# Beryl2000/SE-UNet-AirSeg

Hardware: AMD Instinct MI355X
Metric: voxels/sec SE-UNet fwd+bwd, 128^3 patch (higher is better)
Workload: dtype bf16

## Files before the change

se-unet-airseg_amd/csrc/cat.hip:

```cpp
#include "epilogue.h"
#include <type_traits>

namespace seunet {

template <bool XR>
__device__ __forceinline__ void second_branch(const float (&in8)[8], const float (&wa)[8], const float (&wb)[8], float (&x2)[8]) {
#pragma unroll
  for (int j = 0; j < 8; ++j) x2[j] = XR ? wa[j] * in8[0] + wb[j] * in8[1] : in8[j];
}

template <typename T, int LPV, bool TWO, bool XR>
__global__ void __launch_bounds__(EPI_THREADS)
cat_fwd_kernel(const T* __restrict__ raw, const float* __restrict__ mean, const float* __restrict__ rstd,
               const T* __restrict__ raw2, const float* __restrict__ mean2, const float* __restrict__ rstd2, int C, float slope,
               T* __restrict__ out, long long V, const float* __restrict__ w2x, int xic) {
  SEUNET_EPI_THREAD(LPV);
  float mu[8], rs[8], mu2[8], rs2[8], wa[8], wb[8];
#pragma unroll
  for (int j = 0; j < 8; ++j) {
    mu[j] = mean[n * C + c0 + j]; rs[j] = rstd[n * C + c0 + j];
    mu2[j] = TWO ? mean2[n * C + c0 + j] : 0.f;
    rs2[j] = TWO ? rstd2[n * C + c0 + j] : 0.f;
    wa[j] = XR ? w2x[(c0 + j) * xic] : 0.f;
    wb[j] = (XR && xic > 1) ? w2x[(c0 + j) * xic + 1] : 0.f;
  }
  const long long stride = (long long)P * VPB;
  long long v = (long long)blockIdx.x * VPB + vb;
  Pack8<T> nx, nx2;
  zero8p(nx); zero8p(nx2);
  if (v < V) {
    const long long o = ((long long)n * V + v) * C + c0;
    load8p(raw + o, nx);
    if (TWO) load8p(XR ? raw2 + ((long long)n * V + v) * 8 : raw2 + o, nx2);
  }
  for (; v < V; v += stride) {
    const long long o = ((long long)n * V + v) * C + c0;
    float x[8], in2[8], x2[8], y[8];
    unpack8(nx, x);
    if (TWO) { unpack8(nx2, in2); second_branch<XR>(in2, wa, wb, x2); }
    if (v + stride < V) {
      load8p(raw + o + stride * C, nx);
      if (TWO) load8p(XR ? raw2 + ((long long)n * V + v + stride) * 8 : raw2 + o + stride * C, nx2);
    }
#pragma unroll
    for (int j = 0; j < 8; ++j) y[j] = norm_lrelu(x[j], mu[j], rs[j], slope);
    if (TWO) {
#pragma unroll
      for (int j = 0; j < 8; ++j) y[j] += norm_lrelu(x2[j], mu2[j], rs2[j], slope);
    }
    store8(out + o, y);
  }
}

template <typename T, int LPV>
__global__ void __launch_bounds__(EPI_THREADS)
cat_fwd_pool_kernel(const T* __restrict__ raw, const float* __restrict__ mean, const float* __restrict__ rstd,
                    const T* __restrict__ xin, const float* __restrict__ mean2, const float* __restrict__ rstd2, int C, float slope,
                    T* __restrict__ out, T* __restrict__ pooled, int D, int H, int W, const float* __restrict__ w2x, int xic,
                    unsigned* __restrict__ argmax) {
  SEUNET_EPI_THREAD(LPV);
  float mu[8], rs[8], mu2[8], rs2[8], wa[8], wb[8];
#pragma unroll
  for (int j = 0; j < 8; ++j) {
    mu[j] = mean[n * C + c0 + j]; rs[j] = rstd[n * C + c0 + j];
    mu2[j] = mean2[n * C + c0 + j]; rs2[j] = rstd2[n * C + c0 + j];
    wa[j] = w2x[(c0 + j) * xic];
    wb[j] = xic > 1 ? w2x[(c0 + j) * xic + 1] : 0.f;
  }
  const int Do = D / 2, Ho = H / 2, Wo = W / 2;
  const long long V = (long long)D * H * W, Vo = (long long)Do * Ho * Wo;
  const long long stride = (long long)P * VPB;
  for (long long cv = (long long)blockIdx.x * VPB + vb; cv < Vo; cv += stride) {
    const int xo = (int)(cv % Wo);
    const int yo = (int)((cv / Wo) % Ho);
    const int zo = (int)(cv / ((long long)Wo * Ho));
    const long long v0 = ((long long)(2 * zo) * H + 2 * yo) * W + 2 * xo;
    Pack8<T> px[8], pi[8];
#pragma unroll
    for (int k = 0; k < 8; ++k) {
      const long long v = v0 + ((long long)(k >> 2) * H + ((k >> 1) & 1)) * W + (k & 1);
      load8p(raw + ((long long)n * V + v) * C + c0, px[k]);
      load8p(xin + ((long long)n * V + v) * 8, pi[k]);
    }
    float m[8];
// ... 51 lines not shown
               const T* __restrict__ raw2, const float* __restrict__ mean2, const float* __restrict__ rstd2, int C, float slope,
               const float* __restrict__ m1p, const float* __restrict__ m2p, const float* __restrict__ m1bp,
               const float* __restrict__ m2bp, T* dxhat_out, T* dxhat2_out, double* __restrict__ stat_partial,
               double* __restrict__ stat_partial2, long long V, double* __restrict__ xw_partial, const float* __restrict__ w2x,
               int xic, PoolRef pool, float* __restrict__ gx_out, int gx_acc) {
  static_assert(!XG || (APPLY && XR), "XG: pass B of an XR block only");
  static_assert(!XW || XR, "XW: the weight-gradient sums are formed from the recomputed branch's own input voxel");
  SEUNET_EPI_THREAD(LPV);
  const bool pooled = pool.argmax != nullptr;
  const unsigned* pam = pool.argmax + (long long)n * pool.Vo * (C / 8) + cg;
  const T* pgp = reinterpret_cast<const T*>(pool.g_pool) + (long long)n * pool.Vo * C + c0;
  float mu[8], rs[8], mu2[8], rs2[8], a1[8], a2[8], b1[8], b2[8];
  typedef typename std::conditional<sizeof(T) == 2, float, double>::type SumT;
  SumT s[4][8];
  SumT xw[8][2];
  float wa[8], wb[8];
#pragma unroll
  for (int j = 0; j < 8; ++j) {
    xw[j][0] = xw[j][1] = 0.0;
    wa[j] = XR ? w2x[(c0 + j) * xic] : 0.f;
    wb[j] = (XR && xic > 1) ? w2x[(c0 + j) * xic + 1] : 0.f;
  }
#pragma unroll
  for (int j = 0; j < 8; ++j) {
    mu[j] = mean[n * C + c0 + j]; rs[j] = rstd[n * C + c0 + j];
    mu2[j] = TWO ? mean2[n * C + c0 + j] : 0.f;
    rs2[j] = TWO ? rstd2[n * C + c0 + j] : 0.f;
    a1[j] = APPLY ? m1p[n * C + c0 + j] : 0.f;
    a2[j] = APPLY ? m2p[n * C + c0 + j] : 0.f;
    b1[j] = (APPLY && TWO) ? m1bp[n * C + c0 + j] : 0.f;
    b2[j] = (APPLY && TWO) ? m2bp[n * C + c0 + j] : 0.f;
    s[0][j] = s[1][j] = s[2][j] = s[3][j] = 0.0;
  }
  const long long stride = (long long)P * VPB;
  long long v = (long long)blockIdx.x * VPB + vb;
  Pack8<T> ng, nx, nx2, npg;
  unsigned nam = 0, nkpos = 0;
  zero8p(ng); zero8p(nx); zero8p(nx2); zero8p(npg);
  auto fetch_pool = [&](long long vv) __attribute__((always_inline)) {
    unsigned cv;
    pool_locate(pool, (unsigned)vv, nkpos, cv);
    nam = pam[(long long)cv * (C / 8)];
    load8p(pgp + (long long)cv * C, npg);
  };
  if (v < V) {
    const long long o = ((long long)n * V + v) * C + c0;
    load8p(g_out + o, ng);
    load8p(raw + o, nx);
    if (TWO) load8p(XR ? raw2 + ((long long)n * V + v) * 8 : raw2 + o, nx2);
    if (pooled) fetch_pool(v);
  }
  for (; v < V; v += stride) {
    const long long o = ((long long)n * V + v) * C + c0;
    float gy[8], x[8], in2[8], x2[8], d[8];
    unpack8(ng, gy);
    unpack8(nx, x);
    if (TWO) { unpack8(nx2, in2); second_branch<XR>(in2, wa, wb, x2); }
    if (pooled) {
      float gp[8];
      unpack8(npg, gp);
#pragma unroll
      for (int j = 0; j < 8; ++j) gy[j] += ((nam >> (3 * j)) & 7u) == nkpos ? gp[j] : 0.f;
    }
    if (v + stride < V) {
      load8p(g_out + o + stride * C, ng);
      load8p(raw + o + stride * C, nx);
      if (TWO) load8p(XR ? raw2 + ((long long)n * V + v + stride) * 8 : raw2 + o + stride * C, nx2);
      if (pooled) fetch_pool(v + stride);
    }
#pragma unroll
    for (int j = 0; j < 8; ++j) {
      const float xh = (x[j] - mu[j]) * rs[j];
      d[j] = gy[j] * lrelu_slope(xh, slope);
      if (APPLY) d[j] = rs[j] * (d[j] - a1[j] - xh * a2[j]);
      else { s[0][j] += (SumT)d[j]; s[1][j] += (SumT)d[j] * (SumT)xh; }
    }
    if (TWO) {
      float d2[8];
#pragma unroll
      for (int j = 0; j < 8; ++j) {
        const float xh = (x2[j] - mu2[j]) * rs2[j];
        d2[j] = gy[j] * lrelu_slope(xh, slope);
        if (APPLY) d2[j] = rs2[j] * (d2[j] - b1[j] - xh * b2[j]);
        else { s[2][j] += (SumT)d2[j]; s[3][j] += (SumT)d2[j] * (SumT)xh; }
      }
      if (APPLY && !XR) store8(dxhat2_out + o, d2);
      if (XG) {
        float pa = 0.f, pb = 0.f;
#pragma unroll
        for (int j = 0; j < 8; ++j) { pa = fmaf(d2[j], wa[j], pa); pb = fmaf(d2[j], wb[j], pb); }
#pragma unroll
        for (int off = 1; off < LPV; off <<= 1) { pa += shfl_xor_settled(pa, off); pb += shfl_xor_settled(pb, off); }
        if (cg == 0) {
          float* gp = gx_out + ((long long)n * V + v) * xic;
          gp[0] = gx_acc ? gp[0] + pa : pa;
          if (xic > 1) gp[1] = gx_acc ? gp[1] + pb : pb;
        }
      }
      if (XW && !APPLY) {
#pragma unroll
        for (int j = 0; j < 8; ++j) { xw[j][0] += (SumT)d2[j] * (SumT)in2[0]; xw[j][1] += (SumT)d2[j] * (SumT)in2[1]; }
      }
    }
    if (APPLY) store8(dxhat_out + o, d);
  }
  if (APPLY) return;
  const int wave = threadIdx.x >> 6, lane = threadIdx.x & 63;
  if (XW) {
    __shared__ double redx[4][16][16];
#pragma unroll
    for (int j = 0; j < 8; ++j)
#pragma unroll
      for (int i = 0; i < 2; ++i) {
        const double r = stride_sum_d<LPV>((double)xw[j][i]);
        if (lane < LPV) redx[wave][lane][j * 2 + i] = r;
      }
    __syncthreads();
    double* rec = xw_partial + ((long long)n * P + blockIdx.x) * (C * 2);
    for (int e = threadIdx.x; e < LPV * 16; e += EPI_THREADS) {
      const int gq = e / 16, k = e % 16;
      rec[(gq * 8 + (k >> 1)) * 2 + (k & 1)] = ((redx[0][gq][k] + redx[1][gq][k]) + redx[2][gq][k]) + redx[3][gq][k];
    }
  }
  __shared__ double red[4][16][32];
#pragma unroll
  for (int q = 0; q < 4; ++q)
#pragma unroll
    for (int j = 0; j < 8; ++j) {
      const double r = stride_sum_d<LPV>((double)s[q][j]);
      if (lane < LPV) red[wave][lane][q * 8 + j] = r;
    }
  __syncthreads();
  const long long rec = (long long)n * P + blockIdx.x;
  for (int i = threadIdx.x; i < LPV * 32; i += EPI_THREADS) {
    const int gq = i / 32, k = i % 32, q = k >> 3;
    const double tot = ((red[0][gq][k] + red[1][gq][k]) + red[2][gq][k]) + red[3][gq][k];
    const int c = gq * 8 + (k & 7);
    if (q < 2) stat_partial[(rec * C + c) * 2 + q] = tot;
// ... 248 lines not shown
```

se-unet-airseg_amd/csrc/epilogue.h:

```cpp
#pragma once
#include "seunet_common.h"

namespace seunet {

int epi_partials(Dims d);
int launch_channel_stats(int dtype, const void* t, int C, double* partial, Dims d, hipStream_t s);
int launch_stats_finalize(const double* partial, int slots, int C, int N, long long count,
                          float eps, int mode, float* out_a, float* out_b, hipStream_t s);
struct NormIn { const void* raw; const float* mean; const float* rstd; };
struct SseParams {
  const float* w_se;
  const float* w_se2;
  const float* w_side;
  const float* b_side;
  float slope;
};
struct GateBlock { NormIn a; int C; SseParams p; };
struct SseHead {
  float* side_out;
  float* level_map;
  int level_accumulate;
  const float* head_w;
  const float* drop;
  int drop_stride;
// ... 24 lines not shown
  const float* w2;
  int in_channel;
};
struct CatBlock { NormIn a; Branch2 b; int C; float slope; };
struct PoolOut { void* pooled; unsigned* argmax; };
struct PoolGrad { const unsigned* argmax; const void* g_pool; };
struct CatSums {
  double* stat_partial;
  double* stat_partial2;
  double* xw_partial;
};
struct CatApply {
  const float *m1, *m2, *m1b, *m2b;
  void* dx;
  void* dx2;
  float* gx_out;
  int gx_acc;
};
int launch_cat_fwd(int dtype, const CatBlock& b, void* out, const PoolOut& pool, Dims d, hipStream_t s);
int launch_cat_bwd_sums(int dtype, const CatBlock& b, const void* g_out, const PoolGrad& pool, const CatSums& out, Dims d,
                        hipStream_t s);
int launch_cat_bwd_apply(int dtype, const CatBlock& b, const void* g_out, const PoolGrad& pool, const CatApply& io, Dims d,
                         hipStream_t s);
int xbranch_moment_slots(Dims d);
int launch_xbranch_moments(int dtype, const void* x_in, double* partial, Dims d, hipStream_t s);
int launch_xbranch_stats(const double* partial, int slots, const float* w2, int C, int in_channel, int N, long long count,
                         float eps, float* mean2, float* rstd2, double* moments_out, hipStream_t s);
int launch_cat_xgrad_finalize(const double* xw_partial, const double* stat_partial2, int slots, const double* moments, const float* w2,
                              int C, int in_channel, int N, float eps, float* dw, hipStream_t s);
int launch_xbranch_values(int dtype, const void* x_in, const float* w2, int C, int in_channel, float* out_ncdhw, Dims d, hipStream_t s);

#ifdef __HIPCC__
static constexpr int EPI_THREADS = 256;

template <typename T> __device__ __forceinline__ float round_to(float v) {
  if constexpr (sizeof(T) == 4) return v;
  else return unpack_lo<T>(pack2<T>(v, 0.f));
}

template <typename T> __device__ __forceinline__ float gate_sigmoid(float z) {
  if constexpr (sizeof(T) == 4) return 1.f / (1.f + expf(-z));
  else return __builtin_amdgcn_rcpf(1.f + __builtin_amdgcn_exp2f(-1.44269504088896341f * z));
}

#define SEUNET_EPI_THREAD(LPV)                                \
  const int n = blockIdx.y, P = gridDim.x;                    \
  const int cg = threadIdx.x % LPV, vb = threadIdx.x / LPV;   \
  constexpr int VPB = EPI_THREADS / LPV;                      \
  const int c0 = cg * 8

__device__ __forceinline__ float lrelu(float xh, float slope) { return xh > 0.f ? xh : xh * slope; }
__device__ __forceinline__ float norm_lrelu(float x, float mu, float rs, float slope) { return lrelu((x - mu) * rs, slope); }
__device__ __forceinline__ float lrelu_slope(float xh, float slope) { return xh > 0.f ? 1.f : slope; }

template <typename E, int K> __device__ __forceinline__ E wave4_sum(const E (&red)[4][16][K], int g, int k) {
  return ((red[0][g][k] + red[1][g][k]) + red[2][g][k]) + red[3][g][k];
}
template <typename E, int K> __device__ __forceinline__ E wave4_sum(const E (&red)[4][K], int k) {
  return ((red[0][k] + red[1][k]) + red[2][k]) + red[3][k];
}
template <typename E> __device__ __forceinline__ E wave4_sum(const E (&w)[4]) { return ((w[0] + w[1]) + w[2]) + w[3]; }

template <int K> __device__ __forceinline__ void block_sum(const double (&s)[K], double (&red)[4][K]) {
  const int wave = threadIdx.x >> 6, lane = threadIdx.x & 63;
#pragma unroll
  for (int k = 0; k < K; ++k) {
    double r = s[k];
#pragma unroll
    for (int off = 32; off >= 1; off >>= 1) r += shfl_xor_settled(r, off);
    if (lane == 0) red[wave][k] = r;
  }
  __syncthreads();
}

__device__ __forceinline__ void stats_finalize_body(int idx, const double* __restrict__ partial, int slots, int C, double inv_count,
                                                    float eps, int mode, float* __restrict__ out_a, float* __restrict__ out_b) {
  const int n = idx / C, c = idx % C;
  double s1 = 0.0, s2 = 0.0;
  for (int p = threadIdx.x; p < slots; p += 256) {
    const double* q = partial + (((long long)n * slots + p) * C + c) * 2;
    s1 += q[0];
    s2 += q[1];
// ... 43 lines not shown
```

se-unet-airseg_amd/csrc/epilogue.hip:

```cpp
#include "epilogue.h"

namespace seunet {

int epi_partials(Dims d) {
  long long v = d.vox();
  long long p = v / 128;
  if (p < 1) p = 1;
  if (p > 256) p = 256;
  const long long n = d.N > 0 ? d.N : 1, round = 3 * 256;
  if (n * p >= round) {
    const long long q = (n * p / round) * round / n;
    if (q >= 1) p = q;
  }
  return (int)p;
}

template <typename T, int LPV>
__global__ void __launch_bounds__(EPI_THREADS)
channel_stats_kernel(const T* __restrict__ t, int C, double* __restrict__ partial, long long V) {
  SEUNET_EPI_THREAD(LPV);
  double s1[8], s2[8];
#pragma unroll
  for (int j = 0; j < 8; ++j) { s1[j] = 0.0; s2[j] = 0.0; }
  for (long long v = (long long)blockIdx.x * VPB + vb; v < V; v += (long long)P * VPB) {
    float x[8];
    load8(t + ((long long)n * V + v) * C + c0, x);
#pragma unroll
    for (int j = 0; j < 8; ++j) { s1[j] += (double)x[j]; s2[j] += (double)x[j] * (double)x[j]; }
  }
  __shared__ double red[4][16][16];
  const int wave = threadIdx.x >> 6, lane = threadIdx.x & 63;
#pragma unroll
  for (int j = 0; j < 8; ++j) {
    double a = stride_sum_d<LPV>(s1[j]), b = stride_sum_d<LPV>(s2[j]);
    if (lane < LPV) { red[wave][lane][j] = a; red[wave][lane][8 + j] = b; }
  }
  __syncthreads();
  for (int i = threadIdx.x; i < LPV * 16; i += EPI_THREADS) {
    const int g = i / 16, k = i % 16;
    const double tot = wave4_sum(red, g, k);
    const int c = g * 8 + (k & 7);
    partial[(((long long)n * P + blockIdx.x) * C + c) * 2 + (k >> 3)] = tot;
  }
}

__global__ void __launch_bounds__(256)
stats_finalize_kernel(const double* __restrict__ partial, int slots, int C, int N, double inv_count,
                      float eps, int mode, float* __restrict__ out_a, float* __restrict__ out_b) {
  stats_finalize_body(blockIdx.x, partial, slots, C, inv_count, eps, mode, out_a, out_b);
}

int launch_channel_stats(int dtype, const void* t, int C, double* partial, Dims d, hipStream_t s) {
  if (int e = check_c(C)) return e;
  dim3 grid(epi_partials(d), d.N);
  SEUNET_LPV_SWITCH(C / 8, {
    SEUNET_DTYPE_SWITCH(dtype, channel_stats_kernel<T, LPV><<<grid, EPI_THREADS, 0, s>>>((const T*)t, C, partial, d.vox()));
  });
  SEUNET_LAUNCH_CHECK();
  return 0;
}

int launch_stats_finalize(const double* partial, int slots, int C, int N, long long count, float eps,
// ... 8 lines not shown
```

se-unet-airseg_amd/csrc/gate.hip:

```cpp
#include "epilogue.h"

namespace seunet {

template <typename T, int LPV, bool G2>
__global__ void __launch_bounds__(EPI_THREADS)
sse_fwd_kernel(const T* __restrict__ raw, const float* __restrict__ mean, const float* __restrict__ rstd, int C, SseParams p,
               T* __restrict__ e_out, SseHead head, long long V) {
  SEUNET_EPI_THREAD(LPV);
  float mu[8], rs[8], wse[8], wse2[8], w20[8], w21[8];
#pragma unroll
  for (int j = 0; j < 8; ++j) {
    mu[j] = mean[n * C + c0 + j];
    rs[j] = rstd[n * C + c0 + j];
    wse[j] = p.w_se[c0 + j];
    wse2[j] = G2 ? p.w_se2[c0 + j] : 0.f;
    w20[j] = p.w_side[c0 + j];
    w21[j] = p.w_side[C + c0 + j];
  }
  const float b20 = p.b_side[0], b21 = p.b_side[1], slope = p.slope;
  const bool want_side = head.side_out != nullptr || head.level_map != nullptr;
  float hw0 = 0.f, hw1 = 0.f;
  if (head.level_map) {
    hw0 = head.head_w[0] * (head.drop ? head.drop[n * head.drop_stride + 0] : 1.f);
    hw1 = head.head_w[1] * (head.drop ? head.drop[n * head.drop_stride + 1] : 1.f);
  }
  const long long stride = (long long)P * VPB;
  long long v = (long long)blockIdx.x * VPB + vb;
  Pack8<T> nx;
  zero8p(nx);
  if (v < V) load8p(raw + ((long long)n * V + v) * C + c0, nx);
  for (; v < V; v += stride) {
    const long long vi = (long long)n * V + v;
    float x[8], a[8], e[8];
    unpack8(nx, x);
    if (v + stride < V) load8p(raw + (vi + stride) * C + c0, nx);
    float d1 = 0.f;
#pragma unroll
    for (int j = 0; j < 8; ++j) {
      a[j] = norm_lrelu(x[j], mu[j], rs[j], slope);
      d1 += wse[j] * a[j];
    }
    const float g1 = gate_sigmoid<T>(group_sum<LPV>(d1));
    float d2 = 0.f;
#pragma unroll
    for (int j = 0; j < 8; ++j) {
      e[j] = a[j] * g1;
      d2 += wse2[j] * e[j];
    }
    if (G2) {
      const float g2 = gate_sigmoid<T>(group_sum<LPV>(d2));
#pragma unroll
      for (int j = 0; j < 8; ++j) e[j] *= g2;
    }
    store8(e_out + vi * C + c0, e);
    if (want_side) {
      float s0 = 0.f, s1 = 0.f;
#pragma unroll
      for (int j = 0; j < 8; ++j) { s0 += w20[j] * e[j]; s1 += w21[j] * e[j]; }
      s0 = group_sum<LPV>(s0) + b20;
      s1 = group_sum<LPV>(s1) + b21;
      if (cg == 0) {
        if (head.side_out) { head.side_out[vi * 2] = s0; head.side_out[vi * 2 + 1] = s1; }
        if (head.level_map) {
          const float t = hw0 * s0 + hw1 * s1;
          head.level_map[vi] = head.level_accumulate ? head.level_map[vi] + t : t;
        }
      }
    }
  }
}

template <typename T, int LPV, bool G2, bool APPLY, bool LEVEL>
__global__ void __launch_bounds__(EPI_THREADS, (APPLY || G2) ? 1 : 3)
sse_bwd_kernel(const T* __restrict__ raw, const float* __restrict__ mean, const float* __restrict__ rstd, int C, SseParams p,
               SseBwdIn g, SseHead head, const float* __restrict__ m1p, const float* __restrict__ m2p, T* dxhat_out,
               double* __restrict__ stat_partial, float* __restrict__ pgrad_partial, long long V) {
  SEUNET_EPI_THREAD(LPV);
  float mu[8], rs[8], wse[8], wse2[8], w20[8], w21[8];
#pragma unroll
  for (int j = 0; j < 8; ++j) {
    mu[j] = mean[n * C + c0 + j];
    rs[j] = rstd[n * C + c0 + j];
    wse[j] = p.w_se[c0 + j];
    wse2[j] = G2 ? p.w_se2[c0 + j] : 0.f;
    w20[j] = p.w_side[c0 + j];
    w21[j] = p.w_side[C + c0 + j];
  }
  const float b20 = p.b_side[0], b21 = p.b_side[1], slope = p.slope;
  float dr0 = 1.f, dr1 = 1.f, hw0 = 0.f, hw1 = 0.f;
  if (g.g_level) {
    if (head.drop) { dr0 = head.drop[n * head.drop_stride]; dr1 = head.drop[n * head.drop_stride + 1]; }
    hw0 = head.head_w[0] * dr0;
    hw1 = head.head_w[1] * dr1;
  }
  constexpr bool F64ACC = !APPLY && sizeof(T) == 4;
  __shared__ double acc64[F64ACC ? 16 : 1][F64ACC ? EPI_THREADS : 1];
  float fdx[8], fdxx[8];
  float awse[8], awse2[8], aw20[8], aw21[8], am1[8], am2[8];
  int since_flush = 0;
#pragma unroll
  for (int j = 0; j < 8; ++j) {
    if (F64ACC) acc64[j][threadIdx.x] = acc64[8 + j][threadIdx.x] = 0.0;
    fdx[j] = fdxx[j] = 0.f;
    awse[j] = awse2[j] = aw20[j] = aw21[j] = 0.f;
    am1[j] = APPLY ? m1p[n * C + c0 + j] : 0.f;
    am2[j] = APPLY ? m2p[n * C + c0 + j] : 0.f;
  }
  float adb0 = 0.f, adb1 = 0.f, adh0 = 0.f, adh1 = 0.f;
  float wc[8], sgl = 0.f;
#pragma unroll
  for (int j = 0; j < 8; ++j) wc[j] = w20[j] * hw0 + w21[j] * hw1;

  const long long stride = (long long)P * VPB;
  long long v = (long long)blockIdx.x * VPB + vb;
  Pack8<T> nx, nde;
  float ngl = 0.f, ns0 = 0.f, ns1 = 0.f;
  zero8p(nx); zero8p(nde);
#define SSE_BWD_FETCH(vv)                                                                  \
  do {                                                                                     \
    const long long fi_ = (long long)n * V + (vv);                                         \
    load8p(raw + fi_ * C + c0, nx);                                                        \
    if (g.g_e) load8p(reinterpret_cast<const T*>(g.g_e) + fi_ * C + c0, nde);              \
    if (g.g_level) ngl = g.g_level[fi_];                                                   \
    else if (g.g_side) { ns0 = g.g_side[fi_ * 2]; ns1 = g.g_side[fi_ * 2 + 1]; }           \
  } while (0)
  if (v < V) SSE_BWD_FETCH(v);
  for (; v < V; v += stride) {
    const long long vi = (long long)n * V + v;
    float x[8], xh[8], a[8], b[8], e[8], de[8];
    unpack8(nx, x);
    unpack8(nde, de);
    const float gl = ngl, gs0 = ns0, gs1 = ns1;
    if (v + stride < V) SSE_BWD_FETCH(v + stride);
    float d1 = 0.f;
#pragma unroll
    for (int j = 0; j < 8; ++j) {
      xh[j] = (x[j] - mu[j]) * rs[j];
      a[j] = lrelu(xh[j], slope);
      d1 += wse[j] * a[j];
    }
    const float g1 = gate_sigmoid<T>(group_sum<LPV>(d1));
    float d2 = 0.f;
#pragma unroll
    for (int j = 0; j < 8; ++j) { b[j] = a[j] * g1; d2 += wse2[j] * b[j]; }
    float g2 = 1.f;
    if (G2) g2 = gate_sigmoid<T>(group_sum<LPV>(d2));
#pragma unroll
    for (int j = 0; j < 8; ++j) e[j] = G2 ? b[j] * g2 : b[j];

    float t2 = 0.f;
    if (LEVEL) {
      if (!APPLY) sgl += gl;
#pragma unroll
      for (int j = 0; j < 8; ++j) {
        de[j] += gl * wc[j];
        if (!APPLY) aw20[j] += gl * e[j];
        t2 += de[j] * b[j];
      }
    } else {
      float ds0 = 0.f, ds1 = 0.f;
      if (g.g_level) {
        ds0 = hw0 * gl;
        ds1 = hw1 * gl;
        float s0 = 0.f, s1 = 0.f;
#pragma unroll
        for (int j = 0; j < 8; ++j) { s0 += w20[j] * e[j]; s1 += w21[j] * e[j]; }
        s0 = group_sum<LPV>(s0) + b20;
        s1 = group_sum<LPV>(s1) + b21;
        if (!APPLY && cg == 0) { adh0 += gl * dr0 * s0; adh1 += gl * dr1 * s1; }
      } else if (g.g_side) {
        ds0 = gs0;
        ds1 = gs1;
      }
      if (cg == 0) { adb0 += ds0; adb1 += ds1; }
#pragma unroll
      for (int j = 0; j < 8; ++j) {
        de[j] += w20[j] * ds0 + w21[j] * ds1;
        aw20[j] += ds0 * e[j];
        aw21[j] += ds1 * e[j];
        t2 += de[j] * b[j];
      }
    }
    if (G2) {
      const float q2 = group_sum<LPV>(t2) * g2 * (1.f - g2);
#pragma unroll
      for (int j = 0; j < 8; ++j) {
        awse2[j] += q2 * b[j];
        de[j] = de[j] * g2 + q2 * wse2[j];
      }
    }
    float t1 = 0.f;
#pragma unroll
    for (int j = 0; j < 8; ++j) t1 += de[j] * a[j];
    const float q1 = group_sum<LPV>(t1) * g1 * (1.f - g1);
    float dxh[8];
#pragma unroll
    for (int j = 0; j < 8; ++j) {
      awse[j] += q1 * a[j];
      const float da = de[j] * g1 + q1 * wse[j];
      dxh[j] = da * lrelu_slope(xh[j], slope);
      if (APPLY) {
        dxh[j] = rs[j] * (dxh[j] - am1[j] - xh[j] * am2[j]);
      } else {
        fdx[j] += dxh[j];
        fdxx[j] += dxh[j] * xh[j];
      }
    }
    if (APPLY) store8(dxhat_out + vi * C + c0, dxh);
    else if (F64ACC && ++since_flush == 8) {
      since_flush = 0;
#pragma unroll
      for (int j = 0; j < 8; ++j) {
        acc64[j][threadIdx.x] += (double)fdx[j];
        acc64[8 + j][threadIdx.x] += (double)fdxx[j];
        fdx[j] = fdxx[j] = 0.f;
      }
    }
  }
#undef SSE_BWD_FETCH
  if (APPLY) return;
  if (LEVEL) {
    float h0 = cg == 0 ? b20 * sgl : 0.f, h1 = cg == 0 ? b21 * sgl : 0.f;
#pragma unroll
    for (int j = 0; j < 8; ++j) {
      const float G = aw20[j];
      h0 += w20[j] * G;
      h1 += w21[j] * G;
      aw20[j] = hw0 * G;
      aw21[j] = hw1 * G;
    }
    adh0 = dr0 * h0;
    adh1 = dr1 * h1;
    adb0 = cg == 0 ? hw0 * sgl : 0.f;
    adb1 = cg == 0 ? hw1 * sgl : 0.f;
  }
  double sdx[8], sdxx[8];
#pragma unroll
  for (int j = 0; j < 8; ++j) {
    sdx[j] = (F64ACC ? acc64[j][threadIdx.x] : 0.0) + (double)fdx[j];
    sdxx[j] = (F64ACC ? acc64[8 + j][threadIdx.x] : 0.0) + (double)fdxx[j];
  }

  __shared__ double redd[4][16][16];
  __shared__ float red[4][16][32];
  __shared__ float reds[4][4];
  const int wave = threadIdx.x >> 6, lane = threadIdx.x & 63;
#pragma unroll
  for (int j = 0; j < 8; ++j) {
    const double r0 = stride_sum_d<LPV>(sdx[j]), r1 = stride_sum_d<LPV>(sdxx[j]);
    const float r2 = stride_sum<LPV>(awse[j]), r3 = stride_sum<LPV>(awse2[j]);
    const float r4 = stride_sum<LPV>(aw20[j]), r5 = stride_sum<LPV>(aw21[j]);
    if (lane < LPV) {
// ... 43 lines not shown
__global__ void __launch_bounds__(256)
pgrad_reduce_kernel(const float* __restrict__ pg, int records, int C, float* dw_se, float* dw_se2,
                    float* dw_side, float* db_side, float* dhead_w) {
  pgrad_reduce_body(blockIdx.x, pg, records, C, dw_se, dw_se2, dw_side, db_side, dhead_w);
}
__global__ void __launch_bounds__(256)
gate_bwd_finalize_kernel(const double* __restrict__ partial, int slots, int C, int N, double inv_count, float* __restrict__ m1,
                         float* __restrict__ m2, const float* __restrict__ pg, int records, float* dw_se, float* dw_se2,
                         float* dw_side, float* db_side, float* dhead_w) {
  if ((int)blockIdx.x < N * C) stats_finalize_body(blockIdx.x, partial, slots, C, inv_count, 0.f, 1, m1, m2);
  else pgrad_reduce_body((int)blockIdx.x - N * C, pg, records, C, dw_se, dw_se2, dw_side, db_side, dhead_w);
}

int launch_sse_fwd(int dtype, const GateBlock& b, void* e_out, const SseHead& head, Dims d, hipStream_t s) {
  if (int e = check_c(b.C)) return e;
  dim3 grid(epi_partials(d) * 4, d.N);
  const bool g2 = b.p.w_se2 != nullptr;
  SEUNET_LPV_SWITCH(b.C / 8, {
    SEUNET_DTYPE_SWITCH(dtype, {
      if (g2) sse_fwd_kernel<T, LPV, true><<<grid, EPI_THREADS, 0, s>>>((const T*)b.a.raw, b.a.mean, b.a.rstd, b.C, b.p, (T*)e_out, head, d.vox());
      else sse_fwd_kernel<T, LPV, false><<<grid, EPI_THREADS, 0, s>>>((const T*)b.a.raw, b.a.mean, b.a.rstd, b.C, b.p, (T*)e_out, head, d.vox());
    });
  });
  SEUNET_LAUNCH_CHECK();
  return 0;
}

template <typename T, bool APPLY>
static int sse_bwd_t(const GateBlock& b, const SseBwdIn& g, const SseHead& head, const SseSums& o, const SseApply& a, Dims d,
                     hipStream_t s) {
  dim3 grid(epi_partials(d) * (APPLY ? 4 : 1), d.N);
  const bool g2 = b.p.w_se2 != nullptr;
  const bool level = g.g_level != nullptr;
#define SEUNET_SSE_BWD(G2V, LV) sse_bwd_kernel<T, LPV, G2V, APPLY, LV><<<grid, EPI_THREADS, 0, s>>>((const T*)b.a.raw, b.a.mean, b.a.rstd, b.C, b.p, g, head, a.m1, a.m2, (T*)a.draw_out, o.stat_partial, o.pgrad_partial, d.vox())
  SEUNET_LPV_SWITCH(b.C / 8, {
    if (g2) { if (level) SEUNET_SSE_BWD(true, true); else SEUNET_SSE_BWD(true, false); }
    else { if (level) SEUNET_SSE_BWD(false, true); else SEUNET_SSE_BWD(false, false); }
  });
#undef SEUNET_SSE_BWD
  SEUNET_LAUNCH_CHECK();
  return 0;
}

int launch_sse_bwd_sums(int dtype, const GateBlock& b, const SseBwdIn& g, const SseHead& head, const SseSums& out, Dims d,
                        hipStream_t s) {
  if (int e = check_c(b.C)) return e;
  SEUNET_CHECK(out.stat_partial && out.pgrad_partial, "gate_epilogue_bwd_sums needs the partial buffers");
  SEUNET_DTYPE_SWITCH(dtype, return (sse_bwd_t<T, false>(b, g, head, out, SseApply{}, d, s)));
  return 1;
}

int launch_sse_bwd_apply(int dtype, const GateBlock& b, const SseBwdIn& g, const SseHead& head, const SseApply& io, Dims d,
                         hipStream_t s) {
  if (int e = check_c(b.C)) return e;
  SEUNET_CHECK(io.m1 && io.m2 && io.draw_out, "gate_epilogue_bwd_apply needs m1, m2 and the output tensor");
  SEUNET_DTYPE_SWITCH(dtype, return (sse_bwd_t<T, true>(b, g, head, SseSums{}, io, d, s)));
  return 1;
}

int launch_gate_bwd_finalize(const double* stat_partial, int slots, int C, int N, long long count, float* m1, float* m2,
                             const float* pgrad_partial, int records, float* dw_se, float* dw_se2, float* dw_side,
                             float* db_side, float* dhead_w, hipStream_t s) {
  gate_bwd_finalize_kernel<<<N * C + cdiv(4 * C + 4, 4), 256, 0, s>>>(stat_partial, slots, C, N, 1.0 / (double)count, m1, m2,
                                                                     pgrad_partial, records, dw_se, dw_se2, dw_side, db_side, dhead_w);
  SEUNET_LAUNCH_CHECK();
  return 0;
}

int launch_pgrad_reduce(const float* pgrad_partial, int records, int C, float* dw_se, float* dw_se2, float* dw_side, float* db_side,
                        float* dhead_w, hipStream_t s) {
  pgrad_reduce_kernel<<<cdiv(4 * C + 4, 4), 256, 0, s>>>(pgrad_partial, records, C, dw_se, dw_se2, dw_side, db_side, dhead_w);
  SEUNET_LAUNCH_CHECK();
// ... 5 lines not shown
```

Baseline: 581.3 million.

## Add generic multi-stage voxel prefetch ring and deepen SSE backward-apply prefetch

Introduces a reusable macro-based voxel pipeline holding a ring of prefetched stages, with a steady-state phase and a guarded tail phase. The cat, channel-stats and SSE-forward kernels move onto it at depth 1, which keeps their behaviour close to before but adds register prefetching to channel stats. The SSE-forward kernel now also prefetches the level map it accumulates into. The SSE backward apply kernel for bf16 uses a prefetch depth of 3 when each thread runs enough trips, trading extra registers for more memory loads in flight.

```diff
diff --git a/se-unet-airseg_amd/csrc/cat.hip b/se-unet-airseg_amd/csrc/cat.hip
--- a/se-unet-airseg_amd/csrc/cat.hip
+++ b/se-unet-airseg_amd/csrc/cat.hip
@@ -9,6 +9,8 @@
   for (int j = 0; j < 8; ++j) x2[j] = XR ? wa[j] * in8[0] + wb[j] * in8[1] : in8[j];
 }
 
+constexpr int CAT_FWD_PF = 1;
+constexpr int CAT_BWD_PF = 1;
 template <typename T, int LPV, bool TWO, bool XR>
 __global__ void __launch_bounds__(EPI_THREADS)
 cat_fwd_kernel(const T* __restrict__ raw, const float* __restrict__ mean, const float* __restrict__ rstd,
@@ -24,24 +26,22 @@
     wa[j] = XR ? w2x[(c0 + j) * xic] : 0.f;
     wb[j] = (XR && xic > 1) ? w2x[(c0 + j) * xic + 1] : 0.f;
   }
-  const long long stride = (long long)P * VPB;
-  long long v = (long long)blockIdx.x * VPB + vb;
-  Pack8<T> nx, nx2;
-  zero8p(nx); zero8p(nx2);
-  if (v < V) {
-    const long long o = ((long long)n * V + v) * C + c0;
-    load8p(raw + o, nx);
-    if (TWO) load8p(XR ? raw2 + ((long long)n * V + v) * 8 : raw2 + o, nx2);
-  }
-  for (; v < V; v += stride) {
+  struct Stage {
+    Pack8<T> x, x2;
+    __device__ __forceinline__ void clear() { zero8p(x); zero8p(x2); }
+  };
+#define CAT_FWD_FETCH(w, stage)                                                                       \
+  do {                                                                                                \
+    const long long fo_ = ((long long)n * V + (w)) * C + c0;                                          \
+    load8p(raw + fo_, (stage).x);                                                                     \
+    if (TWO) load8p(XR ? raw2 + ((long long)n * V + (w)) * 8 : raw2 + fo_, (stage).x2);               \
+  } while (0)
+  SEUNET_VOXEL_PIPELINE_BEGIN(CAT_FWD_PF, Stage, (long long)blockIdx.x * VPB + vb, (long long)P * VPB, V, CAT_FWD_FETCH)
     const long long o = ((long long)n * V + v) * C + c0;
     float x[8], in2[8], x2[8], y[8];
-    unpack8(nx, x);
-    if (TWO) { unpack8(nx2, in2); second_branch<XR>(in2, wa, wb, x2); }
-    if (v + stride < V) {
-      load8p(raw + o + stride * C, nx);
-      if (TWO) load8p(XR ? raw2 + ((long long)n * V + v + stride) * 8 : raw2 + o + stride * C, nx2);
-    }
+    unpack8(st.x, x);
+    if (TWO) { unpack8(st.x2, in2); second_branch<XR>(in2, wa, wb, x2); }
+    SEUNET_VOXEL_REFILL(CAT_FWD_FETCH);
 #pragma unroll
     for (int j = 0; j < 8; ++j) y[j] = norm_lrelu(x[j], mu[j], rs[j], slope);
     if (TWO) {
@@ -49,7 +49,8 @@
       for (int j = 0; j < 8; ++j) y[j] += norm_lrelu(x2[j], mu2[j], rs2[j], slope);
     }
     store8(out + o, y);
-  }
+  SEUNET_VOXEL_PIPELINE_END
+#undef CAT_FWD_FETCH
 }
 
 template <typename T, int LPV>
@@ -167,42 +168,38 @@
     b2[j] = (APPLY && TWO) ? m2bp[n * C + c0 + j] : 0.f;
     s[0][j] = s[1][j] = s[2][j] = s[3][j] = 0.0;
   }
-  const long long stride = (long long)P * VPB;
-  long long v = (long long)blockIdx.x * VPB + vb;
-  Pack8<T> ng, nx, nx2, npg;
-  unsigned nam = 0, nkpos = 0;
-  zero8p(ng); zero8p(nx); zero8p(nx2); zero8p(npg);
-  auto fetch_pool = [&](long long vv) __attribute__((always_inline)) {
-    unsigned cv;
-    pool_locate(pool, (unsigned)vv, nkpos, cv);
-    nam = pam[(long long)cv * (C / 8)];
-    load8p(pgp + (long long)cv * C, npg);
+  struct Stage {
+    Pack8<T> g, x, x2, pg;
+    unsigned am, kpos;
+    __device__ __forceinline__ void clear() { zero8p(g); zero8p(x); zero8p(x2); zero8p(pg); am = kpos = 0; }
   };
-  if (v < V) {
-    const long long o = ((long long)n * V + v) * C + c0;
-    load8p(g_out + o, ng);
-    load8p(raw + o, nx);
-    if (TWO) load8p(XR ? raw2 + ((long long)n * V + v) * 8 : raw2 + o, nx2);
-    if (pooled) fetch_pool(v);
-  }
-  for (; v < V; v += stride) {
+#define CAT_BWD_FETCH(w, stage)                                                                       \
+  do {                                                                                                \
+    const long long fo_ = ((long long)n * V + (w)) * C + c0;                                          \
+    load8p(g_out + fo_, (stage).g);                                                                   \
+    load8p(raw + fo_, (stage).x);                                                                     \
+    if (TWO) load8p(XR ? raw2 + ((long long)n * V + (w)) * 8 : raw2 + fo_, (stage).x2);               \
+    if (pooled) {                                                                                     \
+      unsigned cv_;                                                                                   \
+      pool_locate(pool, (unsigned)(w), (stage).kpos, cv_);                                            \
+      (stage).am = pam[(long long)cv_ * (C / 8)];                                                     \
+      load8p(pgp + (long long)cv_ * C, (stage).pg);                                                   \
+    }                                                                                                 \
+  } while (0)
+  SEUNET_VOXEL_PIPELINE_BEGIN(CAT_BWD_PF, Stage, (long long)blockIdx.x * VPB + vb, (long long)P * VPB, V, CAT_BWD_FETCH)
     const long long o = ((long long)n * V + v) * C + c0;
     float gy[8], x[8], in2[8], x2[8], d[8];
-    unpack8(ng, gy);
-    unpack8(nx, x);
-    if (TWO) { unpack8(nx2, in2); second_branch<XR>(in2, wa, wb, x2); }
+    unpack8(st.g, gy);
+    unpack8(st.x, x);
+    if (TWO) { unpack8(st.x2, in2); second_branch<XR>(in2, wa, wb, x2); }
     if (pooled) {
       float gp[8];
-      unpack8(npg, gp);
-#pragma unroll
-      for (int j = 0; j < 8; ++j) gy[j] += ((nam >> (3 * j)) & 7u) == nkpos ? gp[j] : 0.f;
-    }
-    if (v + stride < V) {
-      load8p(g_out + o + stride * C, ng);
-      load8p(raw + o + stride * C, nx);
-      if (TWO) load8p(XR ? raw2 + ((long long)n * V + v + stride) * 8 : raw2 + o + stride * C, nx2);
-      if (pooled) fetch_pool(v + stride);
-    }
+      unpack8(st.pg, gp);
+      const unsigned am = st.am, kpos = st.kpos;
+#pragma unroll
+      for (int j = 0; j < 8; ++j) gy[j] += ((am >> (3 * j)) & 7u) == kpos ? gp[j] : 0.f;
+    }
+    SEUNET_VOXEL_REFILL(CAT_BWD_FETCH);
 #pragma unroll
     for (int j = 0; j < 8; ++j) {
       const float xh = (x[j] - mu[j]) * rs[j];
@@ -238,7 +235,8 @@
       }
     }
     if (APPLY) store8(dxhat_out + o, d);
-  }
+  SEUNET_VOXEL_PIPELINE_END
+#undef CAT_BWD_FETCH
   if (APPLY) return;
   const int wave = threadIdx.x >> 6, lane = threadIdx.x & 63;
   if (XW) {
diff --git a/se-unet-airseg_amd/csrc/epilogue.h b/se-unet-airseg_amd/csrc/epilogue.h
--- a/se-unet-airseg_amd/csrc/epilogue.h
+++ b/se-unet-airseg_amd/csrc/epilogue.h
@@ -80,6 +80,7 @@
 
 #ifdef __HIPCC__
 static constexpr int EPI_THREADS = 256;
+constexpr int EPI_PF_MAX = 3;
 
 template <typename T> __device__ __forceinline__ float round_to(float v) {
   if constexpr (sizeof(T) == 4) return v;
@@ -96,6 +97,36 @@
   const int cg = threadIdx.x % LPV, vb = threadIdx.x / LPV;   \
   constexpr int VPB = EPI_THREADS / LPV;                      \
   const int c0 = cg * 8
+
+#define SEUNET_VOXEL_PIPELINE_BEGIN(PF, STAGE, FIRST, STRIDE, VEND, FETCH)                                             \
+  {                                                                                                                    \
+    constexpr int pf_ = (PF);                                                                                          \
+    static_assert(pf_ >= 1 && pf_ <= EPI_PF_MAX, "prefetch distance");                                                 \
+    const long long stride = (STRIDE), vend_ = (VEND);                                                                 \
+    long long v = (FIRST);                                                                                             \
+    STAGE ring_[pf_];                                                                                                  \
+    _Pragma("unroll") for (int k_ = 0; k_ < pf_; ++k_) ring_[k_].clear();                                              \
+    const bool steady_ = pf_ > 1 && v + (2 * pf_ - 1) * stride < vend_;                                                \
+    _Pragma("unroll") for (int phase_ = pf_ > 1 ? 0 : 1; phase_ < 2; ++phase_) {                                       \
+      if (phase_ == 0 ? steady_ : true) {                                                                              \
+        if (phase_ == 0 || !steady_) {                                                                                 \
+          _Pragma("unroll") for (int k_ = 0; k_ < pf_; ++k_)                                                           \
+            if (phase_ == 0 || v + k_ * stride < vend_) FETCH(v + k_ * stride, ring_[k_]);                             \
+        }                                                                                                              \
+        while (phase_ == 0 ? v + (2 * pf_ - 1) * stride < vend_ : v < vend_) {                                         \
+          _Pragma("unroll") for (int k_ = 0; k_ < pf_; ++k_) {                                                         \
+            if (phase_ == 1 && v >= vend_) break;                                                                      \
+            STAGE& st = ring_[k_];                                                                                     \
+            const bool refill_ = phase_ == 0 || v + pf_ * stride < vend_;
+#define SEUNET_VOXEL_REFILL(FETCH) \
+  if (refill_) FETCH(v + pf_ * stride, st)
+#define SEUNET_VOXEL_PIPELINE_END \
+            v += stride;          \
+          }                       \
+        }                         \
+      }                           \
+    }                             \
+  }
 
 __device__ __forceinline__ float lrelu(float xh, float slope) { return xh > 0.f ? xh : xh * slope; }
 __device__ __forceinline__ float norm_lrelu(float x, float mu, float rs, float slope) { return lrelu((x - mu) * rs, slope); }
diff --git a/se-unet-airseg_amd/csrc/epilogue.hip b/se-unet-airseg_amd/csrc/epilogue.hip
--- a/se-unet-airseg_amd/csrc/epilogue.hip
+++ b/se-unet-airseg_amd/csrc/epilogue.hip
@@ -15,6 +15,7 @@
   return (int)p;
 }
 
+constexpr int STATS_PF = 1;
 template <typename T, int LPV>
 __global__ void __launch_bounds__(EPI_THREADS)
 channel_stats_kernel(const T* __restrict__ t, int C, double* __restrict__ partial, long long V) {
@@ -22,12 +23,19 @@
   double s1[8], s2[8];
 #pragma unroll
   for (int j = 0; j < 8; ++j) { s1[j] = 0.0; s2[j] = 0.0; }
-  for (long long v = (long long)blockIdx.x * VPB + vb; v < V; v += (long long)P * VPB) {
+  struct Stage {
+    Pack8<T> x;
+    __device__ __forceinline__ void clear() { zero8p(x); }
+  };
+#define STATS_FETCH(w, stage) load8p(t + ((long long)n * V + (w)) * C + c0, (stage).x)
+  SEUNET_VOXEL_PIPELINE_BEGIN(STATS_PF, Stage, (long long)blockIdx.x * VPB + vb, (long long)P * VPB, V, STATS_FETCH)
     float x[8];
-    load8(t + ((long long)n * V + v) * C + c0, x);
+    unpack8(st.x, x);
+    SEUNET_VOXEL_REFILL(STATS_FETCH);
 #pragma unroll
     for (int j = 0; j < 8; ++j) { s1[j] += (double)x[j]; s2[j] += (double)x[j] * (double)x[j]; }
-  }
+  SEUNET_VOXEL_PIPELINE_END
+#undef STATS_FETCH
   __shared__ double red[4][16][16];
   const int wave = threadIdx.x >> 6, lane = threadIdx.x & 63;
 #pragma unroll
diff --git a/se-unet-airseg_amd/csrc/gate.hip b/se-unet-airseg_amd/csrc/gate.hip
--- a/se-unet-airseg_amd/csrc/gate.hip
+++ b/se-unet-airseg_amd/csrc/gate.hip
@@ -2,6 +2,9 @@
 
 namespace seunet {
 
+constexpr int SSE_FWD_PF = 1;
+constexpr int SSE_APPLY_PF = 3;
+constexpr int SSE_APPLY_MIN_TRIPS = 4;
 template <typename T, int LPV, bool G2>
 __global__ void __launch_bounds__(EPI_THREADS)
 sse_fwd_kernel(const T* __restrict__ raw, const float* __restrict__ mean, const float* __restrict__ rstd, int C, SseParams p,
@@ -24,16 +27,24 @@
     hw0 = head.head_w[0] * (head.drop ? head.drop[n * head.drop_stride + 0] : 1.f);
     hw1 = head.head_w[1] * (head.drop ? head.drop[n * head.drop_stride + 1] : 1.f);
   }
-  const long long stride = (long long)P * VPB;
-  long long v = (long long)blockIdx.x * VPB + vb;
-  Pack8<T> nx;
-  zero8p(nx);
-  if (v < V) load8p(raw + ((long long)n * V + v) * C + c0, nx);
-  for (; v < V; v += stride) {
+  struct Stage {
+    Pack8<T> x;
+    float lm;
+    __device__ __forceinline__ void clear() { zero8p(x); lm = 0.f; }
+  };
+  const bool add_level = head.level_map != nullptr && head.level_accumulate != 0 && cg == 0;
+#define SSE_FWD_FETCH(w, stage)                                  \
+  do {                                                           \
+    const long long fi_ = (long long)n * V + (w);                \
+    load8p(raw + fi_ * C + c0, (stage).x);                       \
+    if (add_level) (stage).lm = head.level_map[fi_];             \
+  } while (0)
+  SEUNET_VOXEL_PIPELINE_BEGIN(SSE_FWD_PF, Stage, (long long)blockIdx.x * VPB + vb, (long long)P * VPB, V, SSE_FWD_FETCH)
     const long long vi = (long long)n * V + v;
     float x[8], a[8], e[8];
-    unpack8(nx, x);
-    if (v + stride < V) load8p(raw + (vi + stride) * C + c0, nx);
+    unpack8(st.x, x);
+    const float lm = st.lm;
+    SEUNET_VOXEL_REFILL(SSE_FWD_FETCH);
     float d1 = 0.f;
 #pragma unroll
     for (int j = 0; j < 8; ++j) {
@@ -63,14 +74,15 @@
         if (head.side_out) { head.side_out[vi * 2] = s0; head.side_out[vi * 2 + 1] = s1; }
         if (head.level_map) {
           const float t = hw0 * s0 + hw1 * s1;
-          head.level_map[vi] = head.level_accumulate ? head.level_map[vi] + t : t;
+          head.level_map[vi] = head.level_accumulate ? lm + t : t;
         }
       }
     }
-  }
-}
-
-template <typename T, int LPV, bool G2, bool APPLY, bool LEVEL>
+  SEUNET_VOXEL_PIPELINE_END
+#undef SSE_FWD_FETCH
+}
+
+template <typename T, int LPV, bool G2, bool APPLY, bool LEVEL, int PF>
 __global__ void __launch_bounds__(EPI_THREADS, (APPLY || G2) ? 1 : 3)
 sse_bwd_kernel(const T* __restrict__ raw, const float* __restrict__ mean, const float* __restrict__ rstd, int C, SseParams p,
                SseBwdIn g, SseHead head, const float* __restrict__ m1p, const float* __restrict__ m2p, T* dxhat_out,
@@ -111,11 +123,122 @@
 #pragma unroll
   for (int j = 0; j < 8; ++j) wc[j] = w20[j] * hw0 + w21[j] * hw1;
 
-  const long long stride = (long long)P * VPB;
-  long long v = (long long)blockIdx.x * VPB + vb;
-  Pack8<T> nx, nde;
-  float ngl = 0.f, ns0 = 0.f, ns1 = 0.f;
-  zero8p(nx); zero8p(nde);
+#define SSE_BWD_VOXEL                                                                                  \
+    float d1 = 0.f;                                                                                    \
+_Pragma("unroll")                                                                                      \
+    for (int j = 0; j < 8; ++j) {                                                                      \
+      xh[j] = (x[j] - mu[j]) * rs[j];                                                                  \
+      a[j] = lrelu(xh[j], slope);                                                                      \
+      d1 += wse[j] * a[j];                                                                             \
+    }                                                                                                  \
+    const float g1 = gate_sigmoid<T>(group_sum<LPV>(d1));                                              \
+    float d2 = 0.f;                                                                                    \
+_Pragma("unroll")                                                                                      \
+    for (int j = 0; j < 8; ++j) { b[j] = a[j] * g1; d2 += wse2[j] * b[j]; }                            \
+    float g2 = 1.f;                                                                                    \
+    if (G2) g2 = gate_sigmoid<T>(group_sum<LPV>(d2));                                                  \
+_Pragma("unroll")                                                                                      \
+    for (int j = 0; j < 8; ++j) e[j] = G2 ? b[j] * g2 : b[j];                                          \
+                                                                                                       \
+                                              \
+    float t2 = 0.f;                                                                                    \
+    if (LEVEL) {                                                                                       \
+      if (!APPLY) sgl += gl;                                                                           \
+_Pragma("unroll")                                                                                      \
+      for (int j = 0; j < 8; ++j) {                                                                    \
+        de[j] += gl * wc[j];                                                                           \
+        if (!APPLY) aw20[j] += gl * e[j];                                                              \
+        t2 += de[j] * b[j];                                                                            \
+      }                                                                                                \
+    } else {                                                                                           \
+      float ds0 = 0.f, ds1 = 0.f;                                                                      \
+      if (g.g_level) {                                                                                 \
+        ds0 = hw0 * gl;                                                                                \
+        ds1 = hw1 * gl;                                                                                \
+        float s0 = 0.f, s1 = 0.f;                                                                      \
+_Pragma("unroll")                                                                                      \
+        for (int j = 0; j < 8; ++j) { s0 += w20[j] * e[j]; s1 += w21[j] * e[j]; }                      \
+        s0 = group_sum<LPV>(s0) + b20;                                                                 \
+        s1 = group_sum<LPV>(s1) + b21;                                                                 \
+        if (!APPLY && cg == 0) { adh0 += gl * dr0 * s0; adh1 += gl * dr1 * s1; }                       \
+      } else if (g.g_side) {                                                                           \
+        ds0 = gs0;                                                                                     \
+        ds1 = gs1;                                                                                     \
+      }                                                                                                \
+      if (cg == 0) { adb0 += ds0; adb1 += ds1; }                                                       \
+_Pragma("unroll")                                                                                      \
+      for (int j = 0; j < 8; ++j) {                                                                    \
+        de[j] += w20[j] * ds0 + w21[j] * ds1;                                                          \
+        aw20[j] += ds0 * e[j];                                                                         \
+        aw21[j] += ds1 * e[j];                                                                         \
+        t2 += de[j] * b[j];                                                                            \
+      }                                                                                                \
+    }                                                                                                  \
+    if (G2) {                                                \
+      const float q2 = group_sum<LPV>(t2) * g2 * (1.f - g2);                                           \
+_Pragma("unroll")                                                                                      \
+      for (int j = 0; j < 8; ++j) {                                                                    \
+        awse2[j] += q2 * b[j];                                                                         \
+        de[j] = de[j] * g2 + q2 * wse2[j];                                               \
+      }                                                                                                \
+    }                                                                                                  \
+    float t1 = 0.f;                                                                                    \
+_Pragma("unroll")                                                                                      \
+    for (int j = 0; j < 8; ++j) t1 += de[j] * a[j];                                                    \
+    const float q1 = group_sum<LPV>(t1) * g1 * (1.f - g1);    \
+    float dxh[8];                                                                                      \
+_Pragma("unroll")                                                                                      \
+    for (int j = 0; j < 8; ++j) {                                                                      \
+      awse[j] += q1 * a[j];                                                                            \
+      const float da = de[j] * g1 + q1 * wse[j];                                                       \
+      dxh[j] = da * lrelu_slope(xh[j], slope);                                                         \
+      if (APPLY) {                                                                                     \
+        dxh[j] = rs[j] * (dxh[j] - am1[j] - xh[j] * am2[j]);                                           \
+      } else {                                                                                         \
+        fdx[j] += dxh[j];                                                                              \
+        fdxx[j] += dxh[j] * xh[j];                                                                     \
+      }                                                                                                \
+    }                                                                                                  \
+    if (APPLY) store8(dxhat_out + vi * C + c0, dxh);                                                   \
+    else if (F64ACC && ++since_flush == 8) {                                                           \
+      since_flush = 0;                                                                                 \
+_Pragma("unroll")                                                                                      \
+      for (int j = 0; j < 8; ++j) {                                                                    \
+        acc64[j][threadIdx.x] += (double)fdx[j];                                                       \
+        acc64[8 + j][threadIdx.x] += (double)fdxx[j];                                                  \
+        fdx[j] = fdxx[j] = 0.f;                                                                        \
+      }                                                                                                \
+    }
+  if constexpr (APPLY) {
+    struct Stage {
+      Pack8<T> x, de;
+      float gl, s0, s1;
+      __device__ __forceinline__ void clear() { zero8p(x); zero8p(de); gl = s0 = s1 = 0.f; }
+    };
+#define SSE_BWD_FETCH(w, stage)                                                                          \
+  do {                                                                                                   \
+    const long long fi_ = (long long)n * V + (w);                                                        \
+    load8p(raw + fi_ * C + c0, (stage).x);                                                               \
+    if (g.g_e) load8p(reinterpret_cast<const T*>(g.g_e) + fi_ * C + c0, (stage).de);                     \
+    if (g.g_level) (stage).gl = g.g_level[fi_];                                                          \
+    else if (g.g_side) { (stage).s0 = g.g_side[fi_ * 2]; (stage).s1 = g.g_side[fi_ * 2 + 1]; }           \
+  } while (0)
+    SEUNET_VOXEL_PIPELINE_BEGIN(PF, Stage, (long long)blockIdx.x * VPB + vb, (long long)P * VPB, V, SSE_BWD_FETCH)
+      const long long vi = (long long)n * V + v;
+      float x[8], xh[8], a[8], b[8], e[8], de[8];
+      unpack8(st.x, x);
+      unpack8(st.de, de);
+      const float gl = st.gl, gs0 = st.s0, gs1 = st.s1;
+      SEUNET_VOXEL_REFILL(SSE_BWD_FETCH);
+      SSE_BWD_VOXEL
+    SEUNET_VOXEL_PIPELINE_END
+#undef SSE_BWD_FETCH
+  } else {
+    const long long stride = (long long)P * VPB;
+    long long v = (long long)blockIdx.x * VPB + vb;
+    Pack8<T> nx, nde;
+    float ngl = 0.f, ns0 = 0.f, ns1 = 0.f;
+    zero8p(nx); zero8p(nde);
 #define SSE_BWD_FETCH(vv)                                                                  \
   do {                                                                                     \
     const long long fi_ = (long long)n * V + (vv);                                         \
@@ -124,100 +247,19 @@
     if (g.g_level) ngl = g.g_level[fi_];                                                   \
     else if (g.g_side) { ns0 = g.g_side[fi_ * 2]; ns1 = g.g_side[fi_ * 2 + 1]; }           \
   } while (0)
-  if (v < V) SSE_BWD_FETCH(v);
-  for (; v < V; v += stride) {
-    const long long vi = (long long)n * V + v;
-    float x[8], xh[8], a[8], b[8], e[8], de[8];
-    unpack8(nx, x);
-    unpack8(nde, de);
-    const float gl = ngl, gs0 = ns0, gs1 = ns1;
-    if (v + stride < V) SSE_BWD_FETCH(v + stride);
-    float d1 = 0.f;
-#pragma unroll
-    for (int j = 0; j < 8; ++j) {
-      xh[j] = (x[j] - mu[j]) * rs[j];
-      a[j] = lrelu(xh[j], slope);
-      d1 += wse[j] * a[j];
-    }
-    const float g1 = gate_sigmoid<T>(group_sum<LPV>(d1));
-    float d2 = 0.f;
-#pragma unroll
-    for (int j = 0; j < 8; ++j) { b[j] = a[j] * g1; d2 += wse2[j] * b[j]; }
-    float g2 = 1.f;
-    if (G2) g2 = gate_sigmoid<T>(group_sum<LPV>(d2));
-#pragma unroll
-    for (int j = 0; j < 8; ++j) e[j] = G2 ? b[j] * g2 : b[j];
-
-    float t2 = 0.f;
-    if (LEVEL) {
-      if (!APPLY) sgl += gl;
-#pragma unroll
-      for (int j = 0; j < 8; ++j) {
-        de[j] += gl * wc[j];
-        if (!APPLY) aw20[j] += gl * e[j];
-        t2 += de[j] * b[j];
-      }
-    } else {
-      float ds0 = 0.f, ds1 = 0.f;
-      if (g.g_level) {
-        ds0 = hw0 * gl;
-        ds1 = hw1 * gl;
-        float s0 = 0.f, s1 = 0.f;
-#pragma unroll
-        for (int j = 0; j < 8; ++j) { s0 += w20[j] * e[j]; s1 += w21[j] * e[j]; }
-        s0 = group_sum<LPV>(s0) + b20;
-        s1 = group_sum<LPV>(s1) + b21;
-        if (!APPLY && cg == 0) { adh0 += gl * dr0 * s0; adh1 += gl * dr1 * s1; }
-      } else if (g.g_side) {
-        ds0 = gs0;
-        ds1 = gs1;
-      }
-      if (cg == 0) { adb0 += ds0; adb1 += ds1; }
-#pragma unroll
-      for (int j = 0; j < 8; ++j) {
-        de[j] += w20[j] * ds0 + w21[j] * ds1;
-        aw20[j] += ds0 * e[j];
-        aw21[j] += ds1 * e[j];
-        t2 += de[j] * b[j];
-      }
-    }
-    if (G2) {
-      const float q2 = group_sum<LPV>(t2) * g2 * (1.f - g2);
-#pragma unroll
-      for (int j = 0; j < 8; ++j) {
-        awse2[j] += q2 * b[j];
-        de[j] = de[j] * g2 + q2 * wse2[j];
-      }
-    }
-    float t1 = 0.f;
-#pragma unroll
-    for (int j = 0; j < 8; ++j) t1 += de[j] * a[j];
-    const float q1 = group_sum<LPV>(t1) * g1 * (1.f - g1);
-    float dxh[8];
-#pragma unroll
-    for (int j = 0; j < 8; ++j) {
-      awse[j] += q1 * a[j];
-      const float da = de[j] * g1 + q1 * wse[j];
-      dxh[j] = da * lrelu_slope(xh[j], slope);
-      if (APPLY) {
-        dxh[j] = rs[j] * (dxh[j] - am1[j] - xh[j] * am2[j]);
-      } else {
-        fdx[j] += dxh[j];
-        fdxx[j] += dxh[j] * xh[j];
-      }
-    }
-    if (APPLY) store8(dxhat_out + vi * C + c0, dxh);
-    else if (F64ACC && ++since_flush == 8) {
-      since_flush = 0;
-#pragma unroll
-      for (int j = 0; j < 8; ++j) {
-        acc64[j][threadIdx.x] += (double)fdx[j];
-        acc64[8 + j][threadIdx.x] += (double)fdxx[j];
-        fdx[j] = fdxx[j] = 0.f;
-      }
-    }
-  }
+    if (v < V) SSE_BWD_FETCH(v);
+    for (; v < V; v += stride) {
+      const long long vi = (long long)n * V + v;
+      float x[8], xh[8], a[8], b[8], e[8], de[8];
+      unpack8(nx, x);
+      unpack8(nde, de);
+      const float gl = ngl, gs0 = ns0, gs1 = ns1;
+      if (v + stride < V) SSE_BWD_FETCH(v + stride);
+      SSE_BWD_VOXEL
+    }
 #undef SSE_BWD_FETCH
+  }
+#undef SSE_BWD_VOXEL
   if (APPLY) return;
   if (LEVEL) {
     float h0 = cg == 0 ? b20 * sgl : 0.f, h1 = cg == 0 ? b21 * sgl : 0.f;
@@ -327,12 +369,16 @@
   dim3 grid(epi_partials(d) * (APPLY ? 4 : 1), d.N);
   const bool g2 = b.p.w_se2 != nullptr;
   const bool level = g.g_level != nullptr;
-#define SEUNET_SSE_BWD(G2V, LV) sse_bwd_kernel<T, LPV, G2V, APPLY, LV><<<grid, EPI_THREADS, 0, s>>>((const T*)b.a.raw, b.a.mean, b.a.rstd, b.C, b.p, g, head, a.m1, a.m2, (T*)a.draw_out, o.stat_partial, o.pgrad_partial, d.vox())
+  constexpr int DEEP_PF = (APPLY && sizeof(T) == 2) ? SSE_APPLY_PF : 1;
+#define SEUNET_SSE_BWD_PF(G2V, LV, PFV) sse_bwd_kernel<T, LPV, G2V, APPLY, LV, PFV><<<grid, EPI_THREADS, 0, s>>>((const T*)b.a.raw, b.a.mean, b.a.rstd, b.C, b.p, g, head, a.m1, a.m2, (T*)a.draw_out, o.stat_partial, o.pgrad_partial, d.vox())
+#define SEUNET_SSE_BWD(G2V, LV) do { if (deep) SEUNET_SSE_BWD_PF(G2V, LV, DEEP_PF); else SEUNET_SSE_BWD_PF(G2V, LV, 1); } while (0)
   SEUNET_LPV_SWITCH(b.C / 8, {
+    const bool deep = d.vox() / ((long long)grid.x * (EPI_THREADS / LPV)) >= SSE_APPLY_MIN_TRIPS;
     if (g2) { if (level) SEUNET_SSE_BWD(true, true); else SEUNET_SSE_BWD(true, false); }
     else { if (level) SEUNET_SSE_BWD(false, true); else SEUNET_SSE_BWD(false, false); }
   });
 #undef SEUNET_SSE_BWD
+#undef SEUNET_SSE_BWD_PF
   SEUNET_LAUNCH_CHECK();
   return 0;
 }
```

After: 584.2 million (median of 6 runs). No clear change (+0.5%).
